# bioinformatics-centre/kaiju

Hardware: AMD Instinct MI355X
Metric: classified reads/sec (150 bp) (higher is better)
Workload: dtype u64

## Files before the change

### kaiju_amd/csrc/capi.hip

```cpp
#include <algorithm>
#include <chrono>
#include <cstdio>
#include <cstring>
#include <memory>
#include <thread>

#include "capi_internal.h"
#include "host_tables.h"
#include "kj_flow.h"
#include "taxonomy.h"
#include "exact_pass.h"
#include "kj_format.h"
#ifdef KJ_GREEDY3
#include "kj_greedy3.h"
#endif

using namespace kj;

constexpr uint32_t kLocDeferRows = 8;

__device__ __forceinline__ void load_tables(ConstTables &s_ct, const ConstTables *g_ct) {
  const uint32_t *src = reinterpret_cast<const uint32_t *>(g_ct);
  uint32_t *dst = reinterpret_cast<uint32_t *>(&s_ct);
  for (uint32_t i = threadIdx.x; i < sizeof(ConstTables) / 4; i += kBlock) dst[i] = src[i];
  __syncthreads();
}

__global__ void __launch_bounds__(kFragBlock)
k_fragments(const ConstTables *__restrict__ g_ct, Params p, SegTables st, Batch b, SegQueue sq, uint32_t *err,
            uint32_t stage_bytes) {
  __shared__ ConstTables s_ct;
  __shared__ int32_t s_entg[17];
  extern __shared__ __attribute__((aligned(16))) uint8_t s_stage[];
  if (threadIdx.x < 17) s_entg[threadIdx.x] = st.ent_g32[threadIdx.x];
  {
    const uint32_t *src = reinterpret_cast<const uint32_t *>(g_ct);
    uint32_t *dst = reinterpret_cast<uint32_t *>(&s_ct);
    for (uint32_t i = threadIdx.x; i < sizeof(ConstTables) / 4; i += kFragBlock) dst[i] = src[i];
    __syncthreads();
  }
  const uint32_t r = blockIdx.x * kFragBlock + threadIdx.x;
  if (r >= b.n_reads) return;
  uint32_t e = 0;
  build_fragments(s_ct, p, TrigCtx{s_entg, st.ent_locut32}, b, sq, r, &e,
                  stage_bytes ? s_stage + 4 * threadIdx.x : nullptr, 4 * kFragBlock, stage_bytes / 4);
  if (e) atomicOr(err, e);
}

constexpr int kS1Block = 64;
template <bool TRIG, int UNITS = kS1Units>
__global__ void __launch_bounds__(kS1Block)
k_fragments_fast(const Stage1Tables *__restrict__ g_t, Params p, Batch b, SegQueue sq, uint32_t *err) {
  __shared__ __attribute__((aligned(16))) Stage1Tables s_t;
  __shared__ uint32_t s_codes[2 * kS1ListCap * kS1Block];
  __shared__ __attribute__((aligned(4))) uint8_t s_cnt[TRIG ? kS1Block * kS1CntStride : 4];
  {
    const uint4 *src = reinterpret_cast<const uint4 *>(g_t);
    uint4 *dst = reinterpret_cast<uint4 *>(&s_t);
    for (uint32_t i = threadIdx.x; i < sizeof(Stage1Tables) / 16; i += kS1Block) dst[i] = src[i];
    __syncthreads();
  }
  const uint32_t r = blockIdx.x * kS1Block + threadIdx.x;
  if (r >= b.n_reads) return;
  uint32_t e = 0;
  S1Lane ln;
  ln.codes = s_codes + threadIdx.x; ln.code_stride = kS1Block;
  ln.cnt = s_cnt + (TRIG ? threadIdx.x * kS1CntStride : 0);
  ln.tsbuf = nullptr;
  build_fragments_fast<TRIG, UNITS>(s_t, p, b, sq, r, &e, ln);
  if (e) atomicOr(err, e);
}

constexpr int kS1TeamBlock = 256;
constexpr int kS1TeamsPerBlock = kS1TeamBlock / (int)kS1TeamLanes;
__global__ void __launch_bounds__(kS1TeamBlock)
k_fragments_team(const Stage1Tables *__restrict__ g_t, Params p, Batch b, uint32_t *err) {
  __shared__ __attribute__((aligned(16))) Stage1Tables s_t;
  __shared__ __attribute__((aligned(16))) S1TeamLds s_team[kS1TeamsPerBlock];
  {
    const uint4 *src = reinterpret_cast<const uint4 *>(g_t);
    uint4 *dst = reinterpret_cast<uint4 *>(&s_t);
    for (uint32_t i = threadIdx.x; i < sizeof(Stage1Tables) / 16; i += kS1TeamBlock) dst[i] = src[i];
    __syncthreads();
  }
  const uint32_t team = threadIdx.x / kS1TeamLanes;
  const uint32_t r = blockIdx.x * kS1TeamsPerBlock + team;
  if (r >= b.n_reads) return;
  uint32_t e = 0;
  S1TeamDev tm{&s_team[team], threadIdx.x % kS1TeamLanes};
  build_fragments_team(s_t, p, b, r, &e, tm);
  if (e) atomicOr(err, e);
}

__global__ void __launch_bounds__(256)
k_trigcheck(const Stage1Tables *__restrict__ g_t, Params p, Batch b, uint32_t *seglist, uint32_t *segcount) {
  __shared__ __attribute__((aligned(16))) Stage1Tables s_t;
  __shared__ __attribute__((aligned(4))) uint8_t s_cnt[256 * kS1CntStride];
  {
    const uint4 *src = reinterpret_cast<const uint4 *>(g_t);
    uint4 *dst = reinterpret_cast<uint4 *>(&s_t);
    for (uint32_t i = threadIdx.x; i < sizeof(Stage1Tables) / 16; i += 256) dst[i] = src[i];
    __syncthreads();
  }
  const uint32_t r = blockIdx.x * 256 + threadIdx.x;
  if (r >= b.n_reads) return;
  const uint32_t v = b.hits[r].reserved;
  if (v == 0) return;
  b.hits[r].reserved = 0;
  const bool need = lazy_seg_needed(s_t, p, b, r, b.hits + r, v, nullptr, s_cnt + threadIdx.x * kS1CntStride);
  if (need) seglist[atomicAdd(segcount, 1u)] = r;
}
__global__ void __launch_bounds__(256)
k_segflag(Params p, SegTables st, Batch b, SegQueue sq, const uint32_t *seglist, const uint32_t *segcount, uint32_t *err) {
  __shared__ int64_t s_entg[13];
  if (threadIdx.x < 13) s_entg[threadIdx.x] = st.ent_g[threadIdx.x];
  __syncthreads();
  const SegCtx cx = seg_ctx(st, s_entg, nullptr);
  const uint32_t n = *segcount;
  for (uint32_t i = blockIdx.x * 256 + threadIdx.x; i < n; i += gridDim.x * 256) {
    const uint32_t r = seglist[i];
    const ReadMeta rm = b.meta[r];
    Frag *F = b.frags + rm.frag;
    const uint8_t *pep = b.pep + rm.pep;
    const uint32_t nf = rm.nfrag & ~kNfragSegPending;
    uint32_t pending = 0;
    for (uint32_t k = 0; k < nf; k++) {
      const Frag f = F[k];
      uint32_t fl = kFragChecked;
      if (seg_triggers(cx, pep + f.start, (int)f.len)) {
        const uint32_t slot = atomicAdd(sq.count, 1u);
        if (slot >= sq.cap) atomicOr(err, 2u);
        else {
          SegWork wk; wk.read = r; wk.frag = k;
          sq.items[slot] = wk;
          pending = kNfragSegPending;
          fl = (slot + 1) << kFragSlotShift;
        }
      }
      F[k].flags = fl;
    }
    b.meta[r].nfrag = nf | pending;
    uint64_t *h8 = reinterpret_cast<uint64_t *>(b.hits + r);
    for (int x = 0; x < (int)(sizeof(Hit) / 8); x++) h8[x] = 0;
  }
}
__global__ void __launch_bounds__(kBlock)
k_seg_apply_list(const ConstTables *__restrict__ g_ct, Params p, Batch b, SegQueue sq, const uint32_t *seglist,
                 const uint32_t *segcount, uint32_t *err) {
  __shared__ ConstTables s_ct;
  load_tables(s_ct, g_ct);
  const uint32_t n = *segcount;
  uint32_t e = 0;
  for (uint32_t i = blockIdx.x * kBlock + threadIdx.x; i < n; i += gridDim.x * kBlock) seg_apply_mem(s_ct, p, b, sq, seglist[i], &e);
  if (e) atomicOr(err, e);
}

#ifdef KJ_POST_WAVES
#define KJ_POST_BOUNDS __launch_bounds__(256, KJ_POST_WAVES)
#else
#define KJ_POST_BOUNDS __launch_bounds__(256)
#endif
template <bool LCA>
__global__ void KJ_POST_BOUNDS
k_mem_post1(const Stage1Tables *__restrict__ g_t, DevIndex ix, Params p, Batch b, DevTaxonomy t, CompactHit *__restrict__ compact, int lazy,
            uint32_t *seglist, uint32_t *segcount, uint32_t *todo, uint32_t *todocount) {
  __shared__ __attribute__((aligned(16))) Stage1Tables s_t;
  __shared__ __attribute__((aligned(4))) uint8_t s_cnt[256 * kS1CntStride];
  if (lazy) {
    const uint4 *src = reinterpret_cast<const uint4 *>(g_t);
    uint4 *dst = reinterpret_cast<uint4 *>(&s_t);
    for (uint32_t i = threadIdx.x; i < sizeof(Stage1Tables) / 16; i += 256) dst[i] = src[i];
    __syncthreads();
  }
  const uint32_t r = blockIdx.x * 256 + threadIdx.x;
  bool need = false, later = false;
  if (r < b.n_reads) {
    Hit *h = b.hits + r;
    const uint32_t v = lazy ? h->reserved : 0u;
    if (v != 0) {
      h->reserved = 0;
#ifndef KJ_POST_NOTRIG
      need = lazy_seg_needed(s_t, p, b, r, h, v, nullptr, s_cnt + threadIdx.x * kS1CntStride);
#endif
    }
    if (!need) {
      if (h->flags & kHitRetry) later = true;
#ifdef KJ_POST_NOLOCATE
      else if (LCA) { CompactHit ch; ch.lca = 0; ch.best = h->best; ch.info = 0; compact[r] = ch; }
#else
      else if (!mem_locate_read<false>(ix, p, h, kLocDeferRows)) later = true;
      else if (LCA) compact[r] = compact_hit(t, *h);
#endif
    }
  }
  const uint32_t lane = threadIdx.x & 63u;
  {
    const uint64_t m = __ballot(need);
    if (m) {
      const uint32_t leader = (uint32_t)__builtin_ctzll(m);
      uint32_t base = 0;
      if (lane == leader) base = atomicAdd(segcount, (uint32_t)__popcll(m));
      base = (uint32_t)__shfl((int)base, (int)leader, 64);
      if (need) seglist[base + (uint32_t)__popcll(m & ((1ull << lane) - 1ull))] = r;
    }
  }
  {
    const bool td = need || later;
    const uint64_t m = __ballot(td);
    if (m) {
      const uint32_t leader = (uint32_t)__builtin_ctzll(m);
      uint32_t base = 0;
      if (lane == leader) base = atomicAdd(todocount, (uint32_t)__popcll(m));
      base = (uint32_t)__shfl((int)base, (int)leader, 64);
      if (td) todo[base + (uint32_t)__popcll(m & ((1ull << lane) - 1ull))] = r;
    }
  }
}
template <bool LCA>
__global__ void __launch_bounds__(256)
k_mem_post2(DevIndex ix, Params p, Batch b, DevTaxonomy t, CompactHit *__restrict__ compact, const uint32_t *__restrict__ todo,
            const uint32_t *__restrict__ todocount) {
  const uint32_t n = *todocount;
  for (uint32_t i = blockIdx.x * 256 + threadIdx.x; i < n; i += gridDim.x * 256) {
    const uint32_t r = todo[i];
    Hit *h = b.hits + r;
    if (!mem_locate_read<false>(ix, p, h, kLocDeferRows)) mem_locate_read<false, true>(ix, p, h);
    if (LCA) compact[r] = compact_hit(t, *h);
  }
}

__global__ void __launch_bounds__(kFragBlock)
k_fragments_protein(const ConstTables *__restrict__ g_ct, Params p, SegTables st, Batch b, SegQueue sq, uint32_t *err) {
  __shared__ ConstTables s_ct;
  __shared__ int32_t s_entg[17];
  __shared__ uint8_t s_code[256];
  if (threadIdx.x < 17) s_entg[threadIdx.x] = st.ent_g32[threadIdx.x];
  {
    const uint32_t *src = reinterpret_cast<const uint32_t *>(g_ct);
    uint32_t *dst = reinterpret_cast<uint32_t *>(&s_ct);
    for (uint32_t i = threadIdx.x; i < sizeof(ConstTables) / 4; i += kFragBlock) dst[i] = src[i];
    for (uint32_t i = threadIdx.x; i < 256; i += kFragBlock) s_code[i] = 0;
    __syncthreads();
// ... 1629 lines not shown
```

### kaiju_amd/csrc/kj_core.h

```cpp
#pragma once
#include <type_traits>
#include <stdint.h>

#if defined(__HIPCC__)
#include <hip/hip_runtime.h>
#define KJ_HD __host__ __device__ __forceinline__
#define KJ_HD_NOINLINE __host__ __device__ __noinline__
#else
#define KJ_HD inline
#define KJ_HD_NOINLINE inline
struct uint2 { uint32_t x, y; };
struct ulonglong2 { uint64_t x, y; };
#endif

namespace kj {

struct u128 { uint64_t x, y; };
typedef u128 u128_unaligned __attribute__((aligned(1)));
typedef uint32_t u32_unaligned __attribute__((aligned(1)));
typedef uint64_t u64_unaligned __attribute__((aligned(1)));

constexpr int kMaxIds = 21;
constexpr int kSbShift = 16;
constexpr uint32_t kHitIdCap = 1u, kHitSiCap = 2u;
// ... 1430 lines not shown
  for (int i = 0; i < 64; i++) r |= ((v >> i) & 1ull) << (63 - i);
  return r;
#endif
}

KJ_HD uint64_t mk_rev_low(uint64_t m, uint32_t nbits) { return bitrev64(m) >> (64u - nbits); }
KJ_HD Mask128 mk_rev_low(const Mask128 &m, uint32_t nbits) { return mk_shr(Mask128{bitrev64(m.hi), bitrev64(m.lo)}, 128u - nbits); }

KJ_HD uint32_t s1_start(int f, uint32_t u, uint32_t a, uint32_t l) {
  return f < 3 ? (uint32_t)f * (16 * u) + a : (uint32_t)(f + 1) * (16 * u) - a - l;
}

template <class MaskT, class Emit>
KJ_HD void s1_runs(const MaskT *ns, const MaskT *tg, uint32_t len, uint32_t m, uint32_t area, uint32_t seq_base,
                   Emit &&emit) {
  if (m > 64u || m == 0u) return;
  const uint32_t top = len - 3, u = len / 48u + 1u;
  const uint32_t seqF = seq_base, seqR = seq_base + len + 3;
  for (int f = 0; f < 6; f++) {
    const int g = f < 3 ? f : f - 3;
    MaskT E = ns[f];
    uint32_t w = 1;
    while (2 * w <= m) { E = mk_and(E, mk_shr(E, w)); w *= 2; }
    if (w < m) E = mk_and(E, mk_shr(E, m - w));
    while (mk_any(E)) {
      const uint32_t a = mk_ctz(E);
      uint32_t run = 0;
      E = mk_clear_lowest_run(E, run);
      const uint32_t l = run + m - 1;
      uint32_t seq;
      if (f < 3) {
        const uint32_t p = 3 * (a + l) + (uint32_t)g;
        seq = p <= top ? seqF + p : seqF + len + (uint32_t)g;
      } else {
        seq = a == 0 ? seqR + len + (uint32_t)g : seqR + (top - (3 * (a - 1) + (uint32_t)g));
      }
      const bool trig = l >= 12u && mk_range_any(tg[f], a + 11u, l - 11u);
      emit(area + s1_start(f, u, a, l), l, seq, trig);
    }
  }
}

template <bool TRIG, int UNITS = kS1Units>
KJ_HD void build_fragments_fast(const Stage1Tables &t, const Params &p, const Batch &b, const SegQueue &sq, uint32_t r,
                                uint32_t *err_flags, const S1Lane &ln) {
  typedef typename std::conditional<(UNITS <= 4), uint64_t, Mask128>::type MaskT;
  constexpr uint32_t kMaxLen = 48u * (uint32_t)UNITS - 1u;
  static_assert(UNITS == kS1Units || UNITS == kS1UnitsLong, "frame strings of four or six units");
  const uint64_t o0 = b.off[2 * (uint64_t)r], o1 = b.off[2 * (uint64_t)r + 1], o2 = b.off[2 * (uint64_t)r + 2];
  uint32_t len1 = (uint32_t)(o1 - o0), len2 = (uint32_t)(o2 - o1);
  const uint32_t m3 = p.m * 3;
  const uint32_t fbase = (uint32_t)frag_base(b.off, r, p.m);
  Frag *list = b.frags + fbase;
  const uint32_t cap = frag_cap(b.off, r, p.m);
  const uint64_t pbase = pep_base(b.off, r);
  uint32_t n = 0, pending = 0;
  if (len1 > kMaxLen || len2 > kMaxLen) {
    if (err_flags) *err_flags |= kErrReadTooLong;
    len1 = len2 = 0;
  }
  const bool skip = b.paired ? (len1 < m3 && len2 < m3) : (len1 < m3);
  if (!skip) {
    uint8_t *area = b.pep + pbase;
    const uint32_t mate_bytes = len1 >= m3 ? 96u * (len1 / 48u + 1u) : 0u;
    auto emit = [&](uint32_t start, uint32_t l, uint32_t seq, bool trig) {
      uint32_t key = l;
      if (p.mode == 1) {
        key = 0;
        uint32_t x = 0;
        for (; x + 4 <= l; x += 4) {
          const uint32_t w = *reinterpret_cast<const u32_unaligned *>(area + start + x);
          key += (uint32_t)t.diag[w & 255u] + t.diag[(w >> 8) & 255u] + t.diag[(w >> 16) & 255u] + t.diag[w >> 24];
        }
        for (; x < l; x++) key += t.diag[area[start + x]];
        if (key < p.min_score) return;
      }
      if (n >= cap) return;
      if (n < (uint32_t)kS1ListCap) {
        ln.codes[(size_t)(2 * n) * ln.code_stride] = key << 11 | (2047u - seq);
        ln.codes[(size_t)(2 * n + 1) * ln.code_stride] = start << 8 | l << 1 | (trig ? 1u : 0u);
      } else {
        Frag f; f.start = start; f.len = l; f.key = key; f.flags = seq << 1 | (trig ? 1u : 0u);
        list[n] = f;
      }
      n++;
    };
    MaskT ns[6], tg[6];
    for (int f = 0; f < 6; f++) tg[f] = mk_zero(MaskT{});
    auto scan_mate = [&](uint8_t *dst, uint32_t len) {
      const uint32_t u = len / 48u + 1u;
      for (int f = 0; f < 6; f++) {
        const MaskT mm = trig_scan_units<UNITS, MaskT>(t, dst + (size_t)f * 16 * u, u, ln.cnt);
        const MaskT tv = f < 3 ? mm : mk_shl(mk_rev_low(mm, 16 * u), 11);
#pragma unroll
        for (int q = 0; q < 6; q++) if (q == f) tg[q] = tv;
      }
    };
    if (len1 >= m3) {
      s1_mate(t, b.seqs + o0, len1, area, ns);
#ifndef KJ_S1_NOSCAN
      if (TRIG && p.seg) scan_mate(area, len1);
#endif
      s1_runs(ns, tg, len1, p.m, 0, 0, emit);
    }
    if (b.paired && len2 >= m3) {
      s1_mate(t, b.seqs + o1, len2, area + mate_bytes, ns);
      if (TRIG && p.seg) scan_mate(area + mate_bytes, len2);
      s1_runs(ns, tg, len2, p.m, mate_bytes, 2 * len1 + 6, emit);
    }
    auto final_flags = [&](uint32_t trig, uint32_t k) -> uint32_t {
      if (!TRIG || !p.seg) return 0u;
      if (!trig) return kFragChecked;
      const uint32_t slot = append_slot(sq.count);
      if (slot >= sq.cap) { if (err_flags) *err_flags |= 2u; return kFragChecked; }
      SegWork wk; wk.read = r; wk.frag = k;
      sq.items[slot] = wk;
      pending = kNfragSegPending;
      return (slot + 1) << kFragSlotShift;
    };
    if (n <= (uint32_t)kS1ListCap) {
      for (uint32_t k = 0; k < n; k++) {
        const uint32_t hi = ln.codes[(size_t)(2 * k) * ln.code_stride], lo = ln.codes[(size_t)(2 * k + 1) * ln.code_stride];
        uint32_t rank = 0;
        for (uint32_t q = 0; q < n; q++) rank += ln.codes[(size_t)(2 * q) * ln.code_stride] > hi ? 1u : 0u;
        Frag f; f.start = lo >> 8; f.len = (lo >> 1) & 127u; f.key = hi >> 11; f.flags = final_flags(lo & 1u, rank);
        list[rank] = f;
      }
    } else {
      for (uint32_t k = 0; k < (uint32_t)kS1ListCap; k++) {
        const uint32_t hi = ln.codes[(size_t)(2 * k) * ln.code_stride], lo = ln.codes[(size_t)(2 * k + 1) * ln.code_stride];
        Frag f; f.start = lo >> 8; f.len = (lo >> 1) & 127u; f.key = hi >> 11; f.flags = (2047u - (hi & 2047u)) << 1 | (lo & 1u);
        list[k] = f;
      }
      for (uint32_t k = 1; k < n; k++) {
        const Frag f = list[k];
        uint32_t pos = k;
        while (pos > 0 && (list[pos - 1].key < f.key || (list[pos - 1].key == f.key && list[pos - 1].flags > f.flags))) {
          list[pos] = list[pos - 1]; pos--;
        }
        list[pos] = f;
      }
      for (uint32_t k = 0; k < n; k++) list[k].flags = final_flags(list[k].flags & 1u, k);
    }
  }
  ReadMeta rm; rm.pep = pbase; rm.frag = fbase; rm.nfrag = n | pending;
  b.meta[r] = rm;
}

constexpr uint32_t kS1TeamLanes = 16;
struct S1TeamLds {
  u128 str[6 * kS1Units];
  uint64_t ns[6];
  uint32_t hi[kS1ListCap], lo[kS1ListCap];
  uint32_t n, pad[3];
};
static_assert(sizeof(S1TeamLds) % 16 == 0, "S1TeamLds is an array of 16-byte aligned team areas");

struct S1TeamHost {
  static constexpr int kSlots = (int)kS1TeamLanes;
  S1TeamLds *lds;
  KJ_HD uint32_t lane(int s) const { return (uint32_t)s; }
  KJ_HD void sync() const {}
  KJ_HD void sync_memory() const {}
  KJ_HD uint32_t xor1(const uint32_t *v, int s) const { return v[s ^ 1]; }
  KJ_HD uint32_t dword(const uint8_t *s, uint32_t len, int32_t at) const {
    uint32_t v = 0;
    for (int32_t i = 0; i < 4; i++) if (at + i >= 0 && at + i < (int32_t)len) v |= (uint32_t)s[at + i] << (8 * i);
    return v;
  }
};
#if defined(__HIPCC__)
struct S1TeamDev {
  static constexpr int kSlots = 1;
  S1TeamLds *lds;
  uint32_t j;
  KJ_HD uint32_t lane(int) const { return j; }
  KJ_HD void sync() const {
#if defined(__HIP_DEVICE_COMPILE__)
    __builtin_amdgcn_fence(__ATOMIC_RELEASE, "wavefront");
    __builtin_amdgcn_wave_barrier();
    __builtin_amdgcn_fence(__ATOMIC_ACQUIRE, "wavefront");
#endif
  }
  KJ_HD void sync_memory() const {
#if defined(__HIP_DEVICE_COMPILE__)
    __threadfence();
#endif
  }
  KJ_HD uint32_t xor1(const uint32_t *v, int) const {
#if defined(__HIP_DEVICE_COMPILE__)
    return (uint32_t)__builtin_amdgcn_mov_dpp((int)v[0], 0xB1, 0xF, 0xF, false);
#else
    return v[0];
#endif
  }
  KJ_HD uint32_t dword(const uint8_t *s, uint32_t, int32_t at) const { return *reinterpret_cast<const uint32_t *>(s + at); }
};
#endif

KJ_HD uint32_t s1_nz4(uint32_t w) { return (((w + 0x7f7f7f7fu) & 0x80808080u) * 0x00204081u) >> 28; }

template <class Team>
KJ_HD void s1_team_mate(const Stage1Tables &t, const Params &p, const Team &tm, const uint8_t *s, uint32_t len, uint8_t *area,
                        uint32_t off, uint32_t seq_base, Frag *list, uint32_t cap) {
  constexpr int W = Team::kSlots;
  S1TeamLds &L = *tm.lds;
  uint32_t *str32 = reinterpret_cast<uint32_t *>(L.str);
  uint8_t *ns8 = reinterpret_cast<uint8_t *>(L.ns);
  const uint32_t u = len / 48u + 1u;
  uint32_t X[W];
  for (int sl = 0; sl < W; sl++) {
    const uint32_t j = tm.lane(sl), from = 12u * j;
    uint32_t w[4] = {0u, 0u, 0u, 0u};
    if (from < len) {
      const uint32_t a = (uint32_t)(reinterpret_cast<uintptr_t>(s + from) & 3u);
      uint32_t d[5];
#pragma unroll
      for (int k = 0; k < 5; k++) {
        const int32_t at = (int32_t)(from + 4u * (uint32_t)k) - (int32_t)a;
        d[k] = at < (int32_t)len ? tm.dword(s, len, at) : 0u;
      }
#pragma unroll
      for (int k = 0; k < 4; k++) w[k] = (uint32_t)((((uint64_t)d[k + 1] << 32) | d[k]) >> (8u * a));
      const uint32_t v = len - from;
      if (v < 16u) {
#pragma unroll
        for (int k = 0; k < 4; k++) {
          const uint32_t q = 4u * (uint32_t)k;
          w[k] &= q >= v ? 0u : (q + 4u <= v ? 0xffffffffu : (1u << (8u * (v - q))) - 1u);
        }
      }
    }
    uint32_t c[14];
#pragma unroll
    for (int q = 0; q < 14; q++) c[q] = t.nuc3[(w[q >> 2] >> (8 * (q & 3))) & 255u];
    uint32_t x = 0;
#pragma unroll
    for (int g = 0; g < 3; g++) {
      uint32_t F = 0, R = 0;
#pragma unroll
      for (int k = 0; k < 4; k++) {
        const uint32_t idx = c[3 * k + g] << 6 | c[3 * k + g + 1] << 3 | c[3 * k + g + 2];
        F |= (uint32_t)t.tf[idx] << (8 * k);
        R |= (uint32_t)t.tr[idx] << (8 * k);
      }
      x |= s1_nz4(F) << (4 * g) | s1_nz4(R) << (4 * (3 + g));
      if (j < 4u * u) {
        str32[(uint32_t)g * 4u * u + j] = F;
        str32[(uint32_t)(3 + g) * 4u * u + 4u * u - 1u - j] = __builtin_bswap32(R);
      }
    }
    X[sl] = j < 4u * u ? x : 0u;
  }
  for (int sl = 0; sl < W; sl++) {
    const uint32_t j = tm.lane(sl), y = tm.xor1(X, sl);
    if (!(j & 1u)) {
#pragma unroll
      for (int f = 0; f < 6; f++) ns8[8 * f + j / 2u] = (uint8_t)(((X[sl] >> (4 * f)) & 15u) | ((y >> (4 * f)) & 15u) << 4);
    }
  }
  tm.sync();
  const uint32_t m = p.m;
  for (int sl = 0; sl < W; sl++) {
    const uint32_t j = tm.lane(sl);
    for (uint32_t k = j; k < 6u * u; k += kS1TeamLanes) *reinterpret_cast<u128 *>(area + 16u * k) = L.str[k];
    if (j >= 6u || m > 64u || m == 0u) continue;
    const int f = (int)j;
    const uint32_t g = f < 3 ? (uint32_t)f : (uint32_t)f - 3u;
    const uint32_t top = len - 3, seqF = seq_base, seqR = seq_base + len + 3;
    uint64_t E = L.ns[f];
    uint32_t wd = 1;
    while (2 * wd <= m) { E &= E >> wd; wd *= 2; }
    if (wd < m) E &= E >> (m - wd);
    while (E) {
      const uint32_t a = mk_ctz(E);
      uint32_t run = 0;
      E = mk_clear_lowest_run(E, run);
      const uint32_t l = run + m - 1;
      uint32_t seq;
      if (f < 3) {
        const uint32_t ps = 3 * (a + l) + g;
        seq = ps <= top ? seqF + ps : seqF + len + g;
      } else {
        seq = a == 0 ? seqR + len + g : seqR + (top - (3 * (a - 1) + g));
      }
      const uint32_t st = s1_start(f, u, a, l);
      uint32_t key = l;
      if (p.mode == 1) {
        const uint8_t *pep = reinterpret_cast<const uint8_t *>(L.str) + st;
        key = 0;
        for (uint32_t x = 0; x < l; x++) key += t.diag[pep[x]];
        if (key < p.min_score) continue;
      }
      const uint32_t slot = append_slot(&L.n);
      if (slot >= cap) continue;
      if (slot < (uint32_t)kS1ListCap) {
        L.hi[slot] = key << 11 | (2047u - seq);
        L.lo[slot] = (off + st) << 8 | l << 1;
      } else {
        Frag fr; fr.start = off + st; fr.len = l; fr.key = key; fr.flags = seq << 1;
        list[slot] = fr;
      }
    }
  }
  tm.sync();
}

template <class Team>
KJ_HD void build_fragments_team(const Stage1Tables &t, const Params &p, const Batch &b, uint32_t r, uint32_t *err_flags,
                                const Team &tm) {
  constexpr int W = Team::kSlots;
  S1TeamLds &L = *tm.lds;
  const uint64_t o0 = b.off[2 * (uint64_t)r], o1 = b.off[2 * (uint64_t)r + 1], o2 = b.off[2 * (uint64_t)r + 2];
  uint32_t len1 = (uint32_t)(o1 - o0), len2 = (uint32_t)(o2 - o1);
  const uint32_t m3 = p.m * 3;
  const uint32_t fbase = (uint32_t)frag_base(b.off, r, p.m);
  Frag *list = b.frags + fbase;
  const uint32_t cap = frag_cap(b.off, r, p.m);
  const uint64_t pbase = pep_base(b.off, r);
  uint32_t n = 0;
  if (len1 > kS1MaxLen || len2 > kS1MaxLen) {
    if (err_flags) *err_flags |= kErrReadTooLong;
    len1 = len2 = 0;
  }
  const bool skip = b.paired ? (len1 < m3 && len2 < m3) : (len1 < m3);
  if (!skip) {
    for (int sl = 0; sl < W; sl++) if (tm.lane(sl) == 0) L.n = 0;
    tm.sync();
    uint8_t *area = b.pep + pbase;
    const uint32_t mate_bytes = len1 >= m3 ? 96u * (len1 / 48u + 1u) : 0u;
    if (len1 >= m3) s1_team_mate(t, p, tm, b.seqs + o0, len1, area, 0, 0, list, cap);
    if (b.paired && len2 >= m3) s1_team_mate(t, p, tm, b.seqs + o1, len2, area + mate_bytes, mate_bytes, 2 * len1 + 6, list, cap);
    n = L.n < cap ? L.n : cap;
    if (n <= (uint32_t)kS1ListCap) {
      for (int sl = 0; sl < W; sl++) {
        for (uint32_t e = tm.lane(sl); e < n; e += kS1TeamLanes) {
          const uint32_t hi = L.hi[e], lo = L.lo[e];
          uint32_t rank = 0;
          for (uint32_t q = 0; q < n; q++) rank += L.hi[q] > hi ? 1u : 0u;
          Frag f; f.start = lo >> 8; f.len = (lo >> 1) & 127u; f.key = hi >> 11; f.flags = 0;
          list[rank] = f;
        }
      }
    } else {
      tm.sync_memory();
      for (int sl = 0; sl < W; sl++) {
        if (tm.lane(sl) != 0) continue;
        for (uint32_t k = 0; k < (uint32_t)kS1ListCap; k++) {
          Frag f; f.start = L.lo[k] >> 8; f.len = (L.lo[k] >> 1) & 127u; f.key = L.hi[k] >> 11; f.flags = (2047u - (L.hi[k] & 2047u)) << 1;
          list[k] = f;
        }
        for (uint32_t k = 1; k < n; k++) {
          const Frag f = list[k];
          uint32_t pos = k;
          while (pos > 0 && (list[pos - 1].key < f.key || (list[pos - 1].key == f.key && list[pos - 1].flags > f.flags))) {
            list[pos] = list[pos - 1]; pos--;
          }
          list[pos] = f;
        }
        for (uint32_t k = 0; k < n; k++) list[k].flags = 0;
      }
    }
  }
  for (int sl = 0; sl < W; sl++) {
    if (tm.lane(sl) != 0) continue;
    ReadMeta rm; rm.pep = pbase; rm.frag = fbase; rm.nfrag = n;
    b.meta[r] = rm;
  }
}

KJ_HD void protein_code_entry(const ConstTables &t, uint32_t a, uint8_t *tbl) {
  const char letters[21] = "ARNDCQEGHILKMFPSTWYV";
  const uint8_t ch = (uint8_t)letters[a];
  tbl[ch] = tbl[ch | 32u] = t.aa_to_idx[a];
}
KJ_HD void build_fragments_protein(const ConstTables &t, const uint8_t *aa_code, const Params &p, const TrigCtx &tc,
                                   const Batch &b, const SegQueue &sq, uint32_t r, uint32_t *err_flags) {
  const uint64_t o0 = b.off[2 * (uint64_t)r], o1 = b.off[2 * (uint64_t)r + 1];
  const uint32_t len = (uint32_t)(o1 - o0);
  Frag *list = b.frags + frag_base(b.off, r, p.m);
  const uint32_t cap = frag_cap(b.off, r, p.m);
  const uint64_t pbase = pep_base(b.off, r);
  uint8_t *pep = b.pep + pbase;
  uint32_t n = 0, pending = 0;
  if (len >= p.m) {
    NucReader rd;
    rd.open(b.seqs + o0, len);
    uint32_t run_start = 0, run_len = 0, sum = 0, seq = 0;
    bool trig = false;
    TrigWin w;
    trig_reset(w);
    uint64_t wacc = 0;
    for (uint32_t x = 0; x < len; x++) {
      const uint32_t a = aa_code[rd.at(x)];
      wacc |= (uint64_t)a << (8u * (x & 7u));
      if ((x & 7u) == 7u) { *reinterpret_cast<uint64_t *>(pep + (x & ~7u)) = wacc; wacc = 0; }
      if (a) {
        if (run_len == 0) run_start = x;
        run_len++;
        sum += (uint32_t)t.diag_idx[a];
        if (trig_push(w, tc, a, run_len)) trig = true;
      } else {
        emit_run(p, list, n, cap, run_start, run_len, sum, seq++, trig);
        run_len = 0; sum = 0; trig = false;
        trig_reset(w);
      }
    }
    *reinterpret_cast<uint64_t *>(pep + (len & ~7u)) = wacc;
    emit_run(p, list, n, cap, run_start, run_len, sum, seq, trig);
    for (uint32_t k = 1; k < n; k++) {
      const Frag f = list[k];
      uint32_t pos = k;
      while (pos > 0 && (list[pos - 1].key < f.key || (list[pos - 1].key == f.key && list[pos - 1].flags > f.flags))) {
        list[pos] = list[pos - 1]; pos--;
      }
      list[pos] = f;
    }
    for (uint32_t k = 0; k < n; k++) {
      uint32_t fl = 0;
      if (p.seg) {
        fl = kFragChecked;
        if (list[k].flags & 1u) {
          const uint32_t slot = append_slot(sq.count);
          if (slot >= sq.cap) { if (err_flags) *err_flags |= 2u; }
          else {
            SegWork wk; wk.read = r; wk.frag = k;
            sq.items[slot] = wk;
            pending = kNfragSegPending;
            fl = (slot + 1) << kFragSlotShift;
          }
        }
      }
      list[k].flags = fl;
    }
  }
  ReadMeta rm; rm.pep = pbase; rm.frag = (uint32_t)frag_base(b.off, r, p.m); rm.nfrag = n | pending;
  b.meta[r] = rm;
}

KJ_HD void seg_apply_mem(const ConstTables &t, const Params &p, const Batch &b, const SegQueue &sq, uint32_t r,
                         uint32_t *err_flags) {
  const ReadMeta rm = b.meta[r];
  const uint32_t raw = rm.nfrag;
  if (!(raw & kNfragSegPending)) return;
  const uint32_t n_orig = raw & ~kNfragSegPending;
  Frag *list = b.frags + rm.frag;
  const uint32_t cap = frag_cap(b.off, r, p.m);
  const uint8_t *pep = b.pep + rm.pep;
  uint32_t np = 0;
  for (uint32_t k = 0; k < n_orig; k++) {
    const Frag f = list[k];
    const uint32_t slot1 = f.flags >> kFragSlotShift;
    if (!slot1) continue;
    const SegRec rec = sq.recs[slot1 - 1];
    if (rec.overflow && err_flags) *err_flags |= 1u;
    uint32_t cnt = n_orig + np;
    seg_split(t, p, rec, pep, f, FragAppend{list, &cnt, cap});
    np = cnt - n_orig;
    list[k].flags |= kFragRemoved;
  }
  uint32_t w = 0;
  for (uint32_t k = 0; k < n_orig; k++) if (!(list[k].flags & kFragRemoved)) list[w++] = list[k];
  for (uint32_t q = 0; q < np; q++) { const Frag pc = list[n_orig + q]; frag_insert(list, w, cap, pc); }
  b.meta[r].nfrag = w;
}

KJ_HD void seg_apply_mem_big(const ConstTables &t, const Params &p, const Batch &b, const BigSeg &big, uint32_t r) {
  const ReadMeta rm = b.meta[r];
  const uint32_t raw = rm.nfrag;
  if (!(raw & kNfragSegPending)) return;
  const uint32_t n_orig = raw & ~kNfragSegPending;
  Frag *list = b.frags + rm.frag;
  const uint32_t cap = frag_cap(b.off, r, p.m);
  const uint8_t *pep = b.pep + rm.pep;
  uint32_t np = 0;
  for (uint32_t k = 0; k < n_orig; k++) {
    const Frag f = list[k];
    const uint32_t slot1 = f.flags >> kFragSlotShift;
    if (!slot1) continue;
// ... 2737 lines not shown
```

Measured before the change: 483.9 million.

## Spread per-frame run extraction across team lanes and add optional codon lookup

The stage-1 team kernel now computes per-frame run masks and run counts in a first pass and stores them in shared memory. A second pass distributes individual runs across all 16 team lanes through a prefix sum, instead of having only six lanes walk their own frame's runs serially. Behind an opt-in macro, a bit-twiddled nucleotide encoder plus a replicated 64-entry codon table in LDS replaces the nuc3/tf/tr lookups. The boundary dword loads are also clamped rather than branched. The redistribution adds an extra sync and makes each lane skip earlier runs by repeated bit clearing, which costs extra work on long run lists.

```diff
diff --git a/kaiju_amd/csrc/capi.hip b/kaiju_amd/csrc/capi.hip
--- a/kaiju_amd/csrc/capi.hip
+++ b/kaiju_amd/csrc/capi.hip
@@ -77,17 +77,31 @@
 k_fragments_team(const Stage1Tables *__restrict__ g_t, Params p, Batch b, uint32_t *err) {
   __shared__ __attribute__((aligned(16))) Stage1Tables s_t;
   __shared__ __attribute__((aligned(16))) S1TeamLds s_team[kS1TeamsPerBlock];
+#if defined(KJ_S1_CODON_LOOKUP)
+  __shared__ __attribute__((aligned(16))) uint32_t s_cod[kS1CodonEntries * kS1CodonCopies];
+#endif
   {
     const uint4 *src = reinterpret_cast<const uint4 *>(g_t);
     uint4 *dst = reinterpret_cast<uint4 *>(&s_t);
     for (uint32_t i = threadIdx.x; i < sizeof(Stage1Tables) / 16; i += kS1TeamBlock) dst[i] = src[i];
+#if defined(KJ_S1_CODON_LOOKUP)
+    uint4 *cod = reinterpret_cast<uint4 *>(s_cod);
+    for (uint32_t i = threadIdx.x; i < kS1CodonEntries * kS1CodonCopies / 4; i += kS1TeamBlock) {
+      const uint32_t v = s1_codon_entry(*g_t, i / (kS1CodonCopies / 4));
+      cod[i] = make_uint4(v, v, v, v);
+    }
+#endif
     __syncthreads();
   }
   const uint32_t team = threadIdx.x / kS1TeamLanes;
   const uint32_t r = blockIdx.x * kS1TeamsPerBlock + team;
   if (r >= b.n_reads) return;
   uint32_t e = 0;
+#if defined(KJ_S1_CODON_LOOKUP)
+  S1TeamDev tm{&s_team[team], threadIdx.x % kS1TeamLanes, s_cod + threadIdx.x % kS1CodonCopies};
+#else
   S1TeamDev tm{&s_team[team], threadIdx.x % kS1TeamLanes};
+#endif
   build_fragments_team(s_t, p, b, r, &e, tm);
   if (e) atomicOr(err, e);
 }
diff --git a/kaiju_amd/csrc/kj_core.h b/kaiju_amd/csrc/kj_core.h
--- a/kaiju_amd/csrc/kj_core.h
+++ b/kaiju_amd/csrc/kj_core.h
@@ -1606,13 +1606,24 @@
   u128 str[6 * kS1Units];
   uint64_t ns[6];
   uint32_t hi[kS1ListCap], lo[kS1ListCap];
-  uint32_t n, pad[3];
+  uint32_t n;
+  uint32_t runs[2];
+  uint32_t pad;
 };
 static_assert(sizeof(S1TeamLds) % 16 == 0, "S1TeamLds is an array of 16-byte aligned team areas");
+
+constexpr uint32_t kS1CodonEntries = 64, kS1CodonCopies = 32;
+KJ_HD uint32_t s1_codon_entry(const Stage1Tables &t, uint32_t e) {
+  const uint32_t idx = (e & 3u) << 6 | ((e >> 2) & 3u) << 3 | ((e >> 4) & 3u);
+  return (uint32_t)t.tf[idx] | (uint32_t)t.tr[idx] << 16;
+}
 
 struct S1TeamHost {
   static constexpr int kSlots = (int)kS1TeamLanes;
   S1TeamLds *lds;
+  mutable uint32_t cod[kS1CodonEntries];
+  KJ_HD void codon_init(const Stage1Tables &t) const { for (uint32_t e = 0; e < kS1CodonEntries; e++) cod[e] = s1_codon_entry(t, e); }
+  KJ_HD uint32_t codon(uint32_t e) const { return cod[e]; }
   KJ_HD uint32_t lane(int s) const { return (uint32_t)s; }
   KJ_HD void sync() const {}
   KJ_HD void sync_memory() const {}
@@ -1628,6 +1639,11 @@
   static constexpr int kSlots = 1;
   S1TeamLds *lds;
   uint32_t j;
+#if defined(KJ_S1_CODON_LOOKUP)
+  const uint32_t *cod;
+  KJ_HD void codon_init(const Stage1Tables &) const {}
+  KJ_HD uint32_t codon(uint32_t e) const { return cod[e * kS1CodonCopies]; }
+#endif
   KJ_HD uint32_t lane(int) const { return j; }
   KJ_HD void sync() const {
 #if defined(__HIP_DEVICE_COMPILE__)
@@ -1654,13 +1670,28 @@
 
 KJ_HD uint32_t s1_nz4(uint32_t w) { return (((w + 0x7f7f7f7fu) & 0x80808080u) * 0x00204081u) >> 28; }
 
+KJ_HD uint32_t s1_codes4(uint32_t w, uint32_t &bad) {
+  const uint32_t f = w & 0xdfdfdfdfu;
+  const uint32_t b = f | ((f >> 4) & 0x01010101u);
+  const uint32_t z = ((b & 0xe9e9e9e9u) ^ 0x41414141u) | (((b >> 4) ^ ((b >> 2) & ~(b >> 1))) & 0x01010101u);
+  bad = (((((z & 0x7f7f7f7fu) + 0x7f7f7f7fu) | z) & 0x80808080u) * 0x00204081u) >> 28;
+  uint32_t x = (b >> 1) & 0x03030303u;
+  x |= x >> 6;
+  x = (x | x >> 12) & 0xffu;
+  return x ^ ((x >> 1) & 0x55u);
+}
+KJ_HD uint32_t s1_keep4(uint32_t v) {
+  const uint32_t m1 = (v * 0x8421u) & 0x01010101u;
+  return (m1 << 8) - m1;
+}
+
 template <class Team>
 KJ_HD void s1_team_mate(const Stage1Tables &t, const Params &p, const Team &tm, const uint8_t *s, uint32_t len, uint8_t *area,
                         uint32_t off, uint32_t seq_base, Frag *list, uint32_t cap) {
   constexpr int W = Team::kSlots;
   S1TeamLds &L = *tm.lds;
   uint32_t *str32 = reinterpret_cast<uint32_t *>(L.str);
-  uint8_t *ns8 = reinterpret_cast<uint8_t *>(L.ns);
+  uint8_t *ns8 = reinterpret_cast<uint8_t *>(L.ns), *run8 = reinterpret_cast<uint8_t *>(L.runs);
   const uint32_t u = len / 48u + 1u;
   uint32_t X[W];
   for (int sl = 0; sl < W; sl++) {
@@ -1668,11 +1699,12 @@
     uint32_t w[4] = {0u, 0u, 0u, 0u};
     if (from < len) {
       const uint32_t a = (uint32_t)(reinterpret_cast<uintptr_t>(s + from) & 3u);
+      const int32_t last = (int32_t)(len - 1u) - (int32_t)(reinterpret_cast<uintptr_t>(s + (len - 1u)) & 3u);
       uint32_t d[5];
 #pragma unroll
       for (int k = 0; k < 5; k++) {
         const int32_t at = (int32_t)(from + 4u * (uint32_t)k) - (int32_t)a;
-        d[k] = at < (int32_t)len ? tm.dword(s, len, at) : 0u;
+        d[k] = tm.dword(s, len, at < last ? at : last);
       }
 #pragma unroll
       for (int k = 0; k < 4; k++) w[k] = (uint32_t)((((uint64_t)d[k + 1] << 32) | d[k]) >> (8u * a));
@@ -1685,10 +1717,11 @@
         }
       }
     }
+    uint32_t x = 0;
+#if !defined(KJ_S1_CODON_LOOKUP)
     uint32_t c[14];
 #pragma unroll
     for (int q = 0; q < 14; q++) c[q] = t.nuc3[(w[q >> 2] >> (8 * (q & 3))) & 255u];
-    uint32_t x = 0;
 #pragma unroll
     for (int g = 0; g < 3; g++) {
       uint32_t F = 0, R = 0;
@@ -1698,6 +1731,24 @@
         F |= (uint32_t)t.tf[idx] << (8 * k);
         R |= (uint32_t)t.tr[idx] << (8 * k);
       }
+#else
+    uint32_t P = 0, V = 0;
+#pragma unroll
+    for (int k = 0; k < 4; k++) {
+      uint32_t bad;
+      P |= s1_codes4(w[k], bad) << (8 * k);
+      V |= bad << (4 * k);
+    }
+    const uint32_t ok = ~(V | V >> 1 | V >> 2);
+#pragma unroll
+    for (int g = 0; g < 3; g++) {
+      uint32_t e[4];
+#pragma unroll
+      for (int k = 0; k < 4; k++) e[k] = tm.codon((P >> (2 * (3 * k + g))) & 63u);
+      const uint32_t lo = e[0] | e[1] << 8, hi = e[2] | e[3] << 8;
+      const uint32_t keep = s1_keep4((ok >> g) & 0x249u);
+      const uint32_t F = ((lo & 0xffffu) | hi << 16) & keep, R = (lo >> 16 | (hi & 0xffff0000u)) & keep;
+#endif
       x |= s1_nz4(F) << (4 * g) | s1_nz4(R) << (4 * (3 + g));
       if (j < 4u * u) {
         str32[(uint32_t)g * 4u * u + j] = F;
@@ -1718,15 +1769,34 @@
   for (int sl = 0; sl < W; sl++) {
     const uint32_t j = tm.lane(sl);
     for (uint32_t k = j; k < 6u * u; k += kS1TeamLanes) *reinterpret_cast<u128 *>(area + 16u * k) = L.str[k];
-    if (j >= 6u || m > 64u || m == 0u) continue;
-    const int f = (int)j;
-    const uint32_t g = f < 3 ? (uint32_t)f : (uint32_t)f - 3u;
+    if (j >= 6u) continue;
+    uint64_t E = 0;
+    if (m >= 1u && m <= 64u) {
+      E = L.ns[j];
+      uint32_t wd = 1;
+      while (2 * wd <= m) { E &= E >> wd; wd *= 2; }
+      if (wd < m) E &= E >> (m - wd);
+    }
+    L.ns[j] = E;
+    run8[j] = (uint8_t)popc64(E & ~(E << 1));
+  }
+  tm.sync();
+  for (int sl = 0; sl < W; sl++) {
+    const uint32_t j = tm.lane(sl);
+    const uint32_t r03 = L.runs[0], r45 = L.runs[1];
+    uint32_t pre[7];
+    pre[0] = 0;
+#pragma unroll
+    for (int k = 0; k < 6; k++) pre[k + 1] = pre[k] + (((k < 4 ? r03 : r45) >> (8 * (k & 3))) & 255u);
     const uint32_t top = len - 3, seqF = seq_base, seqR = seq_base + len + 3;
-    uint64_t E = L.ns[f];
-    uint32_t wd = 1;
-    while (2 * wd <= m) { E &= E >> wd; wd *= 2; }
-    if (wd < m) E &= E >> (m - wd);
-    while (E) {
+    for (uint32_t pr = j; pr < pre[6]; pr += kS1TeamLanes) {
+      uint32_t fu = 0, first = 0;
+#pragma unroll
+      for (int k = 1; k < 6; k++) if (pr >= pre[k]) { fu = (uint32_t)k; first = pre[k]; }
+      const int f = (int)fu;
+      const uint32_t g = f < 3 ? fu : fu - 3u;
+      uint64_t E = L.ns[f];
+      for (uint32_t q = first; q < pr; q++) E &= E + (E & (~E + 1ull));
       const uint32_t a = mk_ctz(E);
       uint32_t run = 0;
       E = mk_clear_lowest_run(E, run);
@@ -1779,6 +1849,9 @@
   }
   const bool skip = b.paired ? (len1 < m3 && len2 < m3) : (len1 < m3);
   if (!skip) {
+#if defined(KJ_S1_CODON_LOOKUP)
+    tm.codon_init(t);
+#endif
     for (int sl = 0; sl < W; sl++) if (tm.lane(sl) == 0) L.n = 0;
     tm.sync();
     uint8_t *area = b.pep + pbase;
```

Result: no change. 479.3 million (-0.9%).
